# stecrotti/MPSKit.jl

Hardware: AMD Instinct MI355X
Metric: DMRG sweeps/sec + ddAC matvec achieved-TFLOP/s, Heisenberg L=100 D=1024 fp64 (higher is better)
Workload: dtype f64; 1 GPU; Heisenberg S=1/2 FiniteMPS L=100 D=1024 d=2 W=5 fp64, 1-site DMRG sweep (2L-2 site updates), fixed Krylov budget 8 matvecs/site; parallelism=single GPU

## Files before the change

### include/mpsk.h

```cpp
#ifndef MPSK_H
#define MPSK_H
#include <stddef.h>
#include <stdint.h>

#ifdef __cplusplus
extern "C" {
#endif

typedef struct mpsk_ctx mpsk_ctx;
typedef struct mpsk_mposlice mpsk_mposlice;

enum { MPSK_F64 = 0, MPSK_C128 = 1 };
enum { MPSK_OK = 0, MPSK_ERR_INVALID = 1, MPSK_ERR_HIP = 2, MPSK_ERR_UNSUPPORTED = 3, MPSK_ERR_NOMEM = 4 };
enum { MPSK_BLOCK_ZERO = 0, MPSK_BLOCK_SCALAR = 1, MPSK_BLOCK_DENSE = 2 };

int mpsk_version(void);
const char* mpsk_last_error(void);

int mpsk_ctx_create(int device, mpsk_ctx** out);
int mpsk_ctx_destroy(mpsk_ctx* ctx);
int mpsk_ctx_set_stream(mpsk_ctx* ctx, void* hip_stream);
int mpsk_ctx_set_dtype(mpsk_ctx* ctx, int dtype);
int mpsk_ctx_get_stream(mpsk_ctx* ctx, void** hip_stream);
int mpsk_ctx_get_device(mpsk_ctx* ctx, int* device);
// ... 32 lines not shown
                    mpsk_hac** out);
enum { MPSK_HAC_CANONICAL = 1 };
int mpsk_hac_create_ex(mpsk_ctx* ctx, const mpsk_mposlice* H, int Dlo, int Dl, int Dr, const void* GL, const void* GR,
                       int flags, mpsk_hac** out);
int mpsk_hac_apply(mpsk_hac* h, const void* x, int nblk, void* y);
int mpsk_hac_eigsolve_fixed(mpsk_hac* hac, const void* x0, int m, void* const* V, void* scal, void* y, void* first_image);
int mpsk_hac_destroy(mpsk_hac* h);
int mpsk_hac_info(const mpsk_hac* h, int* mode, int* nslabs);
int mpsk_dC(mpsk_ctx* ctx, int W, int Dlo, int Dl, int Dr, const void* GL, const void* GR,
            const void* c, void* y);
int mpsk_dAC2(mpsk_ctx* ctx, const mpsk_mposlice* H1, const mpsk_mposlice* H2, int Dlo, int Dl, int Dr,
              const void* GL, const void* GR, const void* x2, void* y2);

int mpsk_dAC2_product(mpsk_ctx* ctx, const mpsk_mposlice* H1, const mpsk_mposlice* H2, int Dl, int Dm, int Dr,
                      const void* GL, const void* GR, const void* AC, const void* AR, void* Y);
int mpsk_complement_tsvd(mpsk_ctx* ctx, int m, int n, const void* Y, int ldy, const void* QL, int ldql, int pl,
                         const void* QR, int ldqr, int pr, int k, void* U, int ldu, void* S, void* Vt, int ldvt, int* kept);
int mpsk_ctx_complement_stats(mpsk_ctx* ctx, long* n_calls, long* n_subspace, long* n_full);

int mpsk_transfer_left(mpsk_ctx* ctx, const mpsk_mposlice* H, int W, int d, int Dl, int Dr, int Dlb,
                       int Drb, const void* GLin, const void* A, const void* Ab, void* GLout);
int mpsk_transfer_right(mpsk_ctx* ctx, const mpsk_mposlice* H, int W, int d, int Dl, int Dr, int Dlb,
                        int Drb, const void* A, const void* Ab, const void* GRin, void* GRout);
int mpsk_regularize(mpsk_ctx* ctx, int W, int D1, int D2, void* v, const void* lvec, const void* rvec);

int mpsk_qrpos(mpsk_ctx* ctx, int m, int n, const void* A, int lda, void* Q, int ldq, void* R, int ldr);
int mpsk_qrpos2(mpsk_ctx* ctx, int m, int n, const void* A1, int lda1, void* Q1, int ldq1, void* R1, int ldr1,
                const void* A2, int lda2, void* Q2, int ldq2, void* R2, int ldr2);
int mpsk_qrlq_pair(mpsk_ctx* ctx, int m, int n, const void* A1, int lda1, void* Q1, int ldq1, void* R1, int ldr1,
                   const void* A2, int lda2, void* L2, int ldl2, void* Q2, int ldq2);
int mpsk_lqpos(mpsk_ctx* ctx, int m, int n, const void* A, int lda, void* L, int ldl, void* Q, int ldq);
int mpsk_ctx_qr_defer(mpsk_ctx* ctx);
int mpsk_ctx_side_mark(mpsk_ctx* ctx);
int mpsk_ctx_side_begin(mpsk_ctx* ctx);
int mpsk_ctx_side_end(mpsk_ctx* ctx);
int mpsk_qr_commit(mpsk_ctx* ctx, int* redone);
int mpsk_tsvd(mpsk_ctx* ctx, int m, int n, const void* theta, int ldt, void* U, int ldu, void* S, void* Vh,
              int ldv, int max_keep, double trunc_err, int* kept, double* disc_norm);
int mpsk_tsplit(mpsk_ctx* ctx, int m, int n, const void* theta, int ldt, int max_keep, double trunc_err,
                void* AL, int ldal, void* C, int ldc, void* AR, int ldar, void* S, int* kept, double* disc_norm);
int mpsk_cx_embed(mpsk_ctx* ctx, int m, int n, const void* H, int64_t ldh, void* E, int64_t lde);
int mpsk_cx_half(mpsk_ctx* ctx, int m, int n, const void* E, int64_t lde, void* H, int64_t ldh);
int mpsk_gemm(mpsk_ctx* ctx, int transA, int transB, int M, int N, int K, double alpha, const void* A,
              int64_t lda, const void* B, int64_t ldb, double beta, void* C, int64_t ldc);

int mpsk_copy2d(mpsk_ctx* ctx, int rows, int cols, const void* src, int64_t lds, void* dst, int64_t ldd);
// ... 25 lines not shown
```

### mpskit.jl_amd/_lib.py

```python
from __future__ import annotations

import ctypes as C
import os

_HERE = os.path.dirname(os.path.abspath(__file__))
LIB_PATH = os.environ.get("MPSK_LIB") or os.path.join(_HERE, "libmpsk.so")


class MpskError(RuntimeError):
    pass


_lib = None

c_void_pp = C.POINTER(C.c_void_p)
c_int32_p = C.POINTER(C.c_int32)
c_double_p = C.POINTER(C.c_double)

SIGNATURES = {
    "mpsk_ctx_create": [C.c_int, c_void_pp],
    "mpsk_ctx_destroy": [C.c_void_p],
    "mpsk_ctx_set_stream": [C.c_void_p, C.c_void_p],
    "mpsk_ctx_synchronize": [C.c_void_p],
    "mpsk_ctx_workspace_reserve": [C.c_void_p, C.c_size_t],
# ... 15 lines not shown
    "mpsk_mposlice_create_dense": [C.c_void_p, C.c_int, C.c_int, C.c_int, C.c_int, C.c_void_p, c_void_pp],
    "mpsk_mposlice_destroy": [C.c_void_p],
    "mpsk_mposlice_dims": [C.c_void_p, C.POINTER(C.c_int), C.POINTER(C.c_int), C.POINTER(C.c_int)],
    "mpsk_dAC": [C.c_void_p, C.c_void_p, C.c_int, C.c_int, C.c_int, C.c_void_p, C.c_void_p, C.c_void_p,
                 C.c_void_p],
    "mpsk_dAC_blocked": [C.c_void_p, C.c_void_p, C.c_int, C.c_int, C.c_int, C.c_int, C.c_void_p, C.c_void_p,
                         C.c_void_p, C.c_void_p],
    "mpsk_ctx_set_dtype": [C.c_void_p, C.c_int],
    "mpsk_ctx_get_stream": [C.c_void_p, c_void_pp],
    "mpsk_ctx_get_device": [C.c_void_p, C.POINTER(C.c_int)],
    "mpsk_hac_create": [C.c_void_p, C.c_void_p, C.c_int, C.c_int, C.c_int, C.c_void_p, C.c_void_p, c_void_pp],
    "mpsk_hac_create_ex": [C.c_void_p, C.c_void_p, C.c_int, C.c_int, C.c_int, C.c_void_p, C.c_void_p, C.c_int, c_void_pp],
    "mpsk_hac_apply": [C.c_void_p, C.c_void_p, C.c_int, C.c_void_p],
    "mpsk_hac_destroy": [C.c_void_p],
    "mpsk_hac_info": [C.c_void_p, C.POINTER(C.c_int), C.POINTER(C.c_int)],
    "mpsk_dC": [C.c_void_p, C.c_int, C.c_int, C.c_int, C.c_int, C.c_void_p, C.c_void_p, C.c_void_p,
                C.c_void_p],
    "mpsk_dAC2": [C.c_void_p, C.c_void_p, C.c_void_p, C.c_int, C.c_int, C.c_int, C.c_void_p, C.c_void_p,
                  C.c_void_p, C.c_void_p],
    "mpsk_transfer_left": [C.c_void_p, C.c_void_p, C.c_int, C.c_int, C.c_int, C.c_int, C.c_int, C.c_int,
                           C.c_void_p, C.c_void_p, C.c_void_p, C.c_void_p],
    "mpsk_transfer_right": [C.c_void_p, C.c_void_p, C.c_int, C.c_int, C.c_int, C.c_int, C.c_int, C.c_int,
                            C.c_void_p, C.c_void_p, C.c_void_p, C.c_void_p],
    "mpsk_regularize": [C.c_void_p, C.c_int, C.c_int, C.c_int, C.c_void_p, C.c_void_p, C.c_void_p],
    "mpsk_qrpos": [C.c_void_p, C.c_int, C.c_int, C.c_void_p, C.c_int, C.c_void_p, C.c_int, C.c_void_p, C.c_int],
    "mpsk_qrpos2": [C.c_void_p, C.c_int, C.c_int, C.c_void_p, C.c_int, C.c_void_p, C.c_int, C.c_void_p, C.c_int,
                    C.c_void_p, C.c_int, C.c_void_p, C.c_int, C.c_void_p, C.c_int],
    "mpsk_qrlq_pair": [C.c_void_p, C.c_int, C.c_int, C.c_void_p, C.c_int, C.c_void_p, C.c_int, C.c_void_p, C.c_int,
                       C.c_void_p, C.c_int, C.c_void_p, C.c_int, C.c_void_p, C.c_int],
    "mpsk_lqpos": [C.c_void_p, C.c_int, C.c_int, C.c_void_p, C.c_int, C.c_void_p, C.c_int, C.c_void_p, C.c_int],
    "mpsk_tsvd": [C.c_void_p, C.c_int, C.c_int, C.c_void_p, C.c_int, C.c_void_p, C.c_int, C.c_void_p,
                  C.c_void_p, C.c_int, C.c_int, C.c_double, C.POINTER(C.c_int), c_double_p],
    "mpsk_tsplit": [C.c_void_p, C.c_int, C.c_int, C.c_void_p, C.c_int, C.c_int, C.c_double, C.c_void_p, C.c_int,
                    C.c_void_p, C.c_int, C.c_void_p, C.c_int, C.c_void_p, C.POINTER(C.c_int), c_double_p],
    "mpsk_gemm": [C.c_void_p, C.c_int, C.c_int, C.c_int, C.c_int, C.c_int, C.c_double, C.c_void_p,
                  C.c_int64, C.c_void_p, C.c_int64, C.c_double, C.c_void_p, C.c_int64],
    "mpsk_copy2d": [C.c_void_p, C.c_int, C.c_int, C.c_void_p, C.c_int64, C.c_void_p, C.c_int64],
    "mpsk_vdot": [C.c_void_p, C.c_int64, C.c_void_p, C.c_void_p, c_double_p],
    "mpsk_vnrm2": [C.c_void_p, C.c_int64, C.c_void_p, c_double_p],
    "mpsk_vaxpby": [C.c_void_p, C.c_int64, C.c_double, C.c_void_p, C.c_double, C.c_void_p],
    "mpsk_vscal": [C.c_void_p, C.c_int64, C.c_double, C.c_void_p],
    "mpsk_vtimes_i": [C.c_void_p, C.c_int64, C.c_void_p, C.c_void_p],
    "mpsk_vcopy": [C.c_void_p, C.c_int64, C.c_void_p, C.c_void_p],
    "mpsk_vzero": [C.c_void_p, C.c_int64, C.c_void_p],
    "mpsk_vmultidot": [C.c_void_p, C.c_int64, C.c_int, c_void_pp, C.c_void_p, c_double_p],
    "mpsk_vgs_step": [C.c_void_p, C.c_int64, C.c_int, c_void_pp, C.c_void_p, c_double_p],
# ... 95 lines not shown
```

### mpskit.jl_amd/backend.py

```python
from __future__ import annotations

import ctypes as C
import numpy as np

from . import _lib
from ._lib import MpskError, check


def _torch():
    import torch
    return torch


class DTensor:
    __slots__ = ("buf", "shape")

    def __init__(self, buf, shape):
        self.buf = buf
        self.shape = tuple(int(s) for s in shape)

    @property
    def ptr(self):
        return self.buf.data_ptr()

# ... 247 lines not shown
              "mpsk_dAC2_product")
        return y

    def complement_tsvd(self, Y: DTensor, QL: DTensor, QR: DTensor, k: int):
        m, n = Y.shape
        pl = 0 if QL is None else QL.shape[1]
        pr = 0 if QR is None else QR.shape[0]
        kk = max(0, min(int(k), m - pl, n - pr))
        U, S, Vt = self.empty(m, kk), self.empty(kk), self.empty(kk, n)
        kept = C.c_int(-1)
        check(self.lib.mpsk_complement_tsvd(self.ctx, m, n, Y.ptr, m, None if QL is None else QL.ptr, m, pl,
                                            None if QR is None else QR.ptr, max(pr, 1), pr, int(k), U.ptr, m, S.ptr, Vt.ptr,
                                            max(kk, 1), C.byref(kept)), "mpsk_complement_tsvd")
        assert kept.value == kk, (kept.value, kk)
        if kk == 0:
            return None, None, None, 0
        return U, S, Vt, kk

    def complement_stats(self):
        a, b, c = C.c_long(), C.c_long(), C.c_long()
        check(self.lib.mpsk_ctx_complement_stats(self.ctx, C.byref(a), C.byref(b), C.byref(c)), "mpsk_ctx_complement_stats")
        return {"calls": a.value, "subspace": b.value, "full": c.value}

    def transfer_left(self, H, GLin: DTensor, A: DTensor, Ab: DTensor, out: DTensor = None, cplx=False):
        if cplx or getattr(H, "cplx", False):
            Dl, d, Dr = A.shape[0] // 2, A.shape[1], A.shape[2]
            Dlb, Drb = Ab.shape[0] // 2, Ab.shape[2]
            W = GLin.shape[0]
            Wout = H.Wr if H is not None else W
            y = self.empty(Wout, 2 * Drb, Dr) if out is None else out
            if H is None:
                self._set_dtype(True)
            try:
                check(self.lib.mpsk_transfer_left(self.ctx, H.handle if H is not None else None, W, d, Dl, Dr, Dlb, Drb,
                                                  GLin.ptr, A.ptr, Ab.ptr, y.ptr), "mpsk_transfer_left")
            finally:
                if H is None:
                    self._set_dtype(False)
            return y
        Dl, d, Dr = A.shape
        Dlb, _, Drb = Ab.shape
        W = GLin.shape[0]
        Wout = H.Wr if H is not None else W
        y = self.empty(Wout, Drb, Dr) if out is None else out
        check(self.lib.mpsk_transfer_left(self.ctx, H.handle if H is not None else None, W, d, Dl, Dr, Dlb, Drb,
                                          GLin.ptr, A.ptr, Ab.ptr, y.ptr), "mpsk_transfer_left")
        return y

    def transfer_right(self, H, GRin: DTensor, A: DTensor, Ab: DTensor, out: DTensor = None, cplx=False):
        if cplx or getattr(H, "cplx", False):
            Dl, d, Dr = A.shape[0] // 2, A.shape[1], A.shape[2]
            Dlb, Drb = Ab.shape[0] // 2, Ab.shape[2]
            W = GRin.shape[0]
            Wout = H.Wl if H is not None else W
            y = self.empty(Wout, 2 * Dl, Dlb) if out is None else out
            if H is None:
                self._set_dtype(True)
            try:
                check(self.lib.mpsk_transfer_right(self.ctx, H.handle if H is not None else None, W, d, Dl, Dr, Dlb, Drb,
                                                   A.ptr, Ab.ptr, GRin.ptr, y.ptr), "mpsk_transfer_right")
            finally:
                if H is None:
                    self._set_dtype(False)
            return y
        Dl, d, Dr = A.shape
        Dlb, _, Drb = Ab.shape
        W = GRin.shape[0]
        Wout = H.Wl if H is not None else W
        y = self.empty(Wout, Dl, Dlb) if out is None else out
        check(self.lib.mpsk_transfer_right(self.ctx, H.handle if H is not None else None, W, d, Dl, Dr, Dlb, Drb,
                                           A.ptr, Ab.ptr, GRin.ptr, y.ptr), "mpsk_transfer_right")
        return y

    def regularize(self, v: DTensor, lvec: DTensor, rvec: DTensor):
        W, D1, D2 = v.shape
        check(self.lib.mpsk_regularize(self.ctx, W, D1, D2, v.ptr, lvec.ptr, rvec.ptr), "mpsk_regularize")
        return v

    def gemm(self, A: DTensor, B: DTensor, transA=False, transB=False, alpha=1.0, beta=0.0, out: DTensor = None,
             m=None, n=None, k=None, lda=None, ldb=None, ldc=None):
        ar, ac = A.shape
        br, bc = B.shape
        M = (ac if transA else ar) if m is None else m
        K = (ar if transA else ac) if k is None else k
        N = (br if transB else bc) if n is None else n
        c = self.empty(M, N) if out is None else out
        check(self.lib.mpsk_gemm(self.ctx, int(transA), int(transB), M, N, K, float(alpha), A.ptr,
                                 ar if lda is None else lda, B.ptr, br if ldb is None else ldb, float(beta),
                                 c.ptr, M if ldc is None else ldc), "mpsk_gemm")
        return c

    def gemm_raw(self, transA, transB, M, N, K, alpha, a_ptr, lda, b_ptr, ldb, beta, c_ptr, ldc):
# ... 459 lines not shown
```

### mpskit.jl_amd/csrc/mpsk_api.hip

```cpp
#include <hip/hip_runtime.h>
#include <cstdio>
#include <cstdlib>
#include <cstring>
#include <cmath>
#include <algorithm>
#include <map>
#include <string>
#include <vector>
#include "mpsk.h"
#include "mpsk_internal.h"

using namespace mpsk;

static thread_local std::string g_err;
static int fail(int code, const std::string& msg) { g_err = msg; return code; }
#define HIPCHK(expr)                                                                        \
  do {                                                                                      \
    hipError_t e_ = (expr);                                                                 \
    if (e_ != hipSuccess)                                                                   \
      return fail(MPSK_ERR_HIP, std::string(#expr) + ": " + hipGetErrorString(e_));         \
  } while (0)
#define REQUIRE(cond, msg)                                                  \
  do {                                                                      \
    if (!(cond)) return fail(MPSK_ERR_INVALID, std::string(__func__) + ": " + (msg)); \
// ... 1 lines not shown

static constexpr int MPSK_DENSE_MIN_CHID = 8;

struct mpsk_mposlice {
  mpsk_ctx* ctx;
  int Wl, Wr, d;
  int dtype = MPSK_F64;
  std::vector<double> Ofull;
  std::vector<double> Ofull_im;
  MixPlan fwd;
  MixPlan bwd;
  MixPlan rgt;
  double Oi(int w, int t, int s, int v) const {
    return Ofull_im.empty() ? 0.0 : Ofull_im[w + (size_t)Wl * (t + d * (s + (size_t)d * v))];
  }
  std::vector<char> row_used, col_used;
  MixPlan rc;
  std::vector<int> rc_w, rc_s, rc_t;
  int rc_nseg = 0;
  bool jordan = false;
  MixPlan jr, jl;
  std::vector<int> jr_p, jl_p;
  int jr_nseg = 0, jl_nseg = 0;
  double O(int w, int t, int s, int v) const { return Ofull[w + (size_t)Wl * (t + d * (s + (size_t)d * v))]; }
  bool dense = false;
  double* d_Od = nullptr;
  mutable std::map<std::pair<int64_t, int64_t>, int64_t*> dtab;
  double* d_OdR = nullptr;
  mutable std::map<std::pair<int64_t, int64_t>, int64_t*> dtabR;
};

struct PoolBuf { void* p; size_t bytes; bool used; hipStream_t last = nullptr; hipEvent_t ev = nullptr; bool ev_set = false; };

struct mpsk_ctx {
  int device = 0;
  hipStream_t stream = nullptr;
  void* ws = nullptr;
  size_t ws_bytes = 0;
  double* d_scal = nullptr;
  double* d_partial = nullptr;
  double* h_scal = nullptr;
  double* d_coef = nullptr;
  double* h_coef = nullptr;
  hipEvent_t ev_coef = nullptr;
  bool coef_pending = false;
  int dtype = MPSK_F64;
// ... 329 lines not shown
            if (s->O(0, t, si, v) != 0.0) { jr.push_back({p, v, s->O(0, t, si, v)}); r_used[p] = 1; }
          for (int w = 1; w < Wl; ++w)
            if (s->O(w, t, si, Wr - 1) != 0.0) { jl.push_back({p, w, s->O(w, t, si, Wr - 1)}); l_used[p] = 1; }
        }
      auto lists = [&](const std::vector<char>& used, std::vector<int>& out, int& nseg) {
        int empty = -1;
        for (int p = 0; p < d * d; ++p) if (!used[p]) { empty = p; break; }
        for (int t = 0; t < d; ++t) {
          int n = 0;
          for (int si = 0; si < d; ++si) n += used[si + d * t];
          nseg = std::max(nseg, n);
        }
        out.assign((size_t)d * nseg, empty);
        for (int t = 0; t < d; ++t) {
          int k = 0;
          for (int si = 0; si < d; ++si) if (used[si + d * t]) out[(size_t)t * nseg + k++] = si + d * t;
        }
      };
      lists(r_used, s->jr_p, s->jr_nseg);
      lists(l_used, s->jl_p, s->jl_nseg);
      HIPCHK(mix_plan_create(jr, d * d, Wr, &s->jr));
      HIPCHK(mix_plan_create(jl, d * d, Wl, &s->jl));
      s->jordan = s->jr_nseg > 0 && s->jl_nseg > 0;
    }
  }
  if (dense) {
    const int Wl = s->Wl, Wr = s->Wr;
    std::vector<double> od((size_t)d * Wl * d * Wr);
    for (int v = 0; v < Wr; ++v)
      for (int t = 0; t < d; ++t)
        for (int w = 0; w < Wl; ++w)
          for (int si = 0; si < d; ++si)
            od[(si + (size_t)d * w) + (size_t)d * Wl * (t + (size_t)d * v)] = s->O(w, t, si, v);
    s->dense = true;
    if (hipMalloc(&s->d_Od, sizeof(double) * od.size()) != hipSuccess) { mpsk_mposlice_destroy(s); return fail(MPSK_ERR_NOMEM, "dense MPO hipMalloc failed"); }
    HIPCHK(hipMemcpy(s->d_Od, od.data(), sizeof(double) * od.size(), hipMemcpyHostToDevice));
    for (int v = 0; v < Wr; ++v)
      for (int t = 0; t < d; ++t)
        for (int w = 0; w < Wl; ++w)
          for (int si = 0; si < d; ++si)
            od[(si + (size_t)d * v) + (size_t)d * Wr * (t + (size_t)d * w)] = s->O(w, t, si, v);
    if (hipMalloc(&s->d_OdR, sizeof(double) * od.size()) != hipSuccess) { mpsk_mposlice_destroy(s); return fail(MPSK_ERR_NOMEM, "dense MPO hipMalloc failed"); }
    HIPCHK(hipMemcpy(s->d_OdR, od.data(), sizeof(double) * od.size(), hipMemcpyHostToDevice));
  }
  *out = s;
  return MPSK_OK;
// ... 10 lines not shown
  REQUIRE(dtype == MPSK_F64, "dense MPO slices are MPSK_F64 only (complex DenseMPO is not implemented; build an MPSK_C128 "
                             "slice with mpsk_mposlice_create instead)");
  REQUIRE(Wl > 0 && Wr > 0 && d > 0, "Wl, Wr and d must be positive");
  const int32_t cl = Wl, cr = Wr, kind = MPSK_BLOCK_DENSE;
  const void* blocks[1] = {O};
  return mposlice_build(c, dtype, 1, &cl, &cr, d, &kind, nullptr, blocks, true, out);
}

int mpsk_mposlice_destroy(mpsk_mposlice* s) {
  if (!s) return MPSK_OK;
  mpsk_ctx* c = s->ctx;
  (void)hipSetDevice(c->device);
  (void)hipStreamSynchronize(c->stream);
  for (auto it = c->pair_plans.begin(); it != c->pair_plans.end();) {
    if (it->first.first == s || it->first.second == s) { mix_plan_destroy(&it->second); it = c->pair_plans.erase(it); }
    else ++it;
  }
  mix_plan_destroy(&s->fwd);
  mix_plan_destroy(&s->bwd);
  mix_plan_destroy(&s->rgt);
  mix_plan_destroy(&s->rc);
  mix_plan_destroy(&s->jr);
  mix_plan_destroy(&s->jl);
  if (s->d_Od) (void)hipFree(s->d_Od);
  if (s->d_OdR) (void)hipFree(s->d_OdR);
  for (auto& kv : s->dtab) (void)hipFree(kv.second);
  for (auto& kv : s->dtabR) (void)hipFree(kv.second);
  delete s;
  return MPSK_OK;
}

int mpsk_mposlice_dims(const mpsk_mposlice* s, int* Wl, int* Wr, int* d) {
  REQUIRE(s, "slice is NULL");
  if (Wl) *Wl = s->Wl;
  if (Wr) *Wr = s->Wr;
  if (d) *d = s->d;
  return MPSK_OK;
}

}

static int ensure_ws(mpsk_ctx* c, size_t bytes) {
  if (c->pend.active) return fail(MPSK_ERR_INVALID, "a deferred factorization still owns the workspace: call mpsk_qr_commit first");
  if (c->on_side) return fail(MPSK_ERR_INVALID, "workspace users are not accepted on the side stream: call mpsk_ctx_side_end first");
  if (bytes <= c->ws_bytes) return MPSK_OK;
  return mpsk_ctx_workspace_reserve(c, bytes + bytes / 4);
// ... 665 lines not shown
  HIPCHK(hipSetDevice(c->device));
  const int d1 = H1->d, d2 = H2->d, Wl = H1->Wl, Wr = H2->Wr;
  const size_t plane = (size_t)Dlo * d1 * Dr;
  const size_t slab = plane * d2;
  if (int rc = ensure_ws(c, sizeof(double) * slab * (Wl + Wr))) return rc;
  double* T1 = (double*)c->ws;
  double* T2 = T1 + slab * Wl;
  const MixPlan* plan = nullptr;
  if (int rc = pair_plan(c, H1, H2, &plan)) return rc;
  GemmArgs g1 = mk((const double*)GL, (const double*)x2, T1, Dlo, d1 * Dr * d2, Dl, Dlo, Dl, Dlo);
  g1.batch = Wl; g1.bsA = (int64_t)Dlo * Dl; g1.bsB = 0; g1.bsC = (int64_t)slab;
  g1.tag = 1;
  HIPCHK(gemm_f64(g1, c->stream));
  SlabIndex ix{d1, d2, (int64_t)Dlo, (int64_t)plane, (int64_t)slab, (int64_t)Dlo * d1};
  HIPCHK(mix_apply(*plan, T1, ix, T2, ix, Dlo, Dr, c->stream));
  std::vector<int64_t> sa, sb;
  for (int v = 0; v < Wr; ++v) if (H2->col_used[v]) { sa.push_back((int64_t)v * slab); sb.push_back((int64_t)v * Dr * Dr); }
  if (sa.empty()) { HIPCHK(zero_async(y2, sizeof(double) * slab, c->stream)); return MPSK_OK; }
  GemmArgs g3 = mk(T2, (const double*)GR, (double*)y2, Dlo * d1, Dr, Dr, (int64_t)Dlo * d1, Dr, (int64_t)Dlo * d1);
  g3.tag = 1;
  g3.batch = d2; g3.bsA = (int64_t)plane; g3.bsB = 0; g3.bsC = (int64_t)plane;
  HIPCHK(gemm_segments(g3, sa, sb, c->stream));
  return MPSK_OK;
}

int mpsk_transfer_left(mpsk_ctx* c, const mpsk_mposlice* H, int W, int d, int Dl, int Dr, int Dlb, int Drb,
                       const void* GLin, const void* A, const void* Ab, void* GLout) {
  REQUIRE(c && GLin && A && Ab && GLout, "NULL argument");
  HIPCHK(hipSetDevice(c->device));
  int Wl = W, Wr = W;
  if (H) { Wl = H->Wl; Wr = H->Wr; d = H->d; }
  REQUIRE(Wl > 0 && d > 0 && Dl > 0 && Dr > 0 && Dlb > 0 && Drb > 0, "dimensions must be positive");
  if ((H ? H->dtype : c->dtype) == MPSK_C128)
    return transfer_left_c128(c, H, W, d, Dl, Dr, Dlb, Drb, (const double*)GLin, (const double*)A, (const double*)Ab, (double*)GLout);
  if (dense_route(H))
    return transfer_left_dense(c, H, Dl, Dr, Dlb, Drb, (const double*)GLin, (const double*)A, (const double*)Ab, (double*)GLout);
  const size_t slab = (size_t)Dlb * d * Dr;
  if (int rc = ensure_ws(c, sizeof(double) * slab * (Wl + (H ? Wr : 0)))) return rc;
  double* T1 = (double*)c->ws;
  double* T2 = H ? T1 + slab * Wl : T1;
  GemmArgs g1 = mk((const double*)GLin, (const double*)A, T1, Dlb, d * Dr, Dl, Dlb, Dl, Dlb);
  g1.batch = Wl; g1.bsA = (int64_t)Dlb * Dl; g1.bsB = 0; g1.bsC = (int64_t)slab;
  HIPCHK(gemm_f64(g1, c->stream));
  if (H) {
    SlabIndex ix{d, 1 << 30, (int64_t)Dlb, (int64_t)slab, 0, (int64_t)Dlb * d};
    HIPCHK(mix_apply(H->fwd, T1, ix, T2, ix, Dlb, Dr, c->stream));
// ... 1563 lines not shown
```

### mpskit.jl_amd/csrc/mpsk_internal.h

```cpp
#pragma once
#include <hip/hip_runtime.h>
#include <stdint.h>
#include <stddef.h>
#include <atomic>
#include <vector>
#include <string>

namespace mpsk {

inline hipError_t ensure_dyn_smem(std::atomic<uint64_t>& done, const void* kernel, size_t bytes) {
  int dev = 0;
  hipError_t e = hipGetDevice(&dev);
  if (e != hipSuccess) return e;
  const uint64_t bit = 1ull << (dev & 63);
  if (done.load(std::memory_order_acquire) & bit) return hipSuccess;
  e = hipFuncSetAttribute(kernel, hipFuncAttributeMaxDynamicSharedMemorySize, (int)bytes);
  if (e != hipSuccess) return e;
  done.fetch_or(bit, std::memory_order_release);
  return hipSuccess;
}

constexpr int MAXSEG = 32;

struct GemmArgs {
// ... 41 lines not shown
std::string gemm_prof_summary();

struct MixTerm { int32_t out, in; double coef; double coef_im = 0.0; };

struct MixPlan {
  int n_out = 0, n_in = 0;
  int32_t* d_rowptr = nullptr;
  int32_t* d_src = nullptr;
  double* d_coef = nullptr;
  double* d_coef_im = nullptr;
  int nnz = 0;
  int max_terms = 0;
};

hipError_t mix_plan_create(const std::vector<MixTerm>& terms, int n_out, int n_in, MixPlan* plan);
void mix_plan_destroy(MixPlan* plan);

struct SlabIndex { int n0, n1; int64_t s0, s1, s2; int64_t ld; };
hipError_t mix_apply(const MixPlan& plan, const double* in, SlabIndex iin, double* out, SlabIndex iout,
                     int R, int C, hipStream_t s);
hipError_t deinterleave(const double* z, int64_t n, double* re, double* im, hipStream_t s);
hipError_t copy_strided(const double* src, int64_t srs, int64_t scs, double* dst, int64_t drs, int64_t dcs, int64_t R,
                        int64_t C, hipStream_t s);

constexpr int MPSK_DOT_SCRATCH = 32 * 1024;
hipError_t vec_multidot(const double* const* xs, int k, const double* y, int64_t n, double* d_out,
                        double* d_partial, hipStream_t s);
hipError_t vec_axpby(double a, const double* x, double b, double* y, int64_t n, hipStream_t s);
hipError_t vec_times_i(const double* x, double* y, int64_t n, hipStream_t s);
hipError_t vec_scal(double a, double* x, int64_t n, hipStream_t s);
hipError_t vec_scal_rsqrt_dev(const double* d_n2, double* x, int64_t n, hipStream_t s);
hipError_t vec_scal_rsqrt_dev_oop(const double* d_n2, const double* x, double* y, int64_t n, hipStream_t s);
hipError_t vec_cgs2(const double* const* xs, int k, double* y, int64_t n, double* d_out, double* d_partial, hipStream_t s);
hipError_t vec_ritz_small(const double* d_slot, int m, int stride, double* d_coef, double* d_info, hipStream_t s);
hipError_t vec_multilincomb(const double* const* xs, int k, double* const* ys, int m, const double* d_coefs, int64_t n,
                            hipStream_t s);
hipError_t vec_multiaxpy(const double* const* xs, const double* d_coefs, int k, double sign, double* y,
                         int64_t n, hipStream_t s);

size_t regularize_workspace_doubles(int W, int D1, int D2);
hipError_t regularize(int W, int D1, int D2, double* v, const double* lvec, const double* rvec, double* partial, hipStream_t s);
hipError_t transpose(const double* in, int ldi, int rows, int cols, double* out, int ldo, hipStream_t s);
size_t qrpos_workspace_doubles(int m, int n);
hipError_t qrpos(int m, int n, const double* A, int lda, double* Q, int ldq, double* R, int ldr, double* ws,
                 hipStream_t s, std::string* err);

// ... 23 lines not shown
```

### mpskit.jl_amd/csrc/mpsk_ops.hip

```cpp
#include <hip/hip_runtime.h>
#include "mpsk_internal.h"

namespace mpsk {

typedef double d2 __attribute__((ext_vector_type(2)));

__device__ inline int64_t slab_off(const SlabIndex& ix, int j) {
  int j0 = j % ix.n0;
  int t = j / ix.n0;
  int j1 = t % ix.n1;
  int j2 = t / ix.n1;
  return j0 * ix.s0 + j1 * ix.s1 + j2 * ix.s2;
}

template <bool VEC2>
__global__ __launch_bounds__(256) void mix_kernel(const int32_t* __restrict__ rowptr,
                                                  const int32_t* __restrict__ src,
                                                  const double* __restrict__ coef,
                                                  const double* __restrict__ coef_im,
                                                  const double* __restrict__ in, SlabIndex iin,
                                                  double* __restrict__ out, SlabIndex iout, int R, int C) {
  const int o = blockIdx.y;
  const int t0 = rowptr[o], t1 = rowptr[o + 1];
  double* op = out + slab_off(iout, o);
// ... 105 lines not shown
}
__global__ __launch_bounds__(256) void deinterleave_kernel(const d2* __restrict__ z, double* __restrict__ re,
                                                           double* __restrict__ im, int64_t n) {
  for (int64_t e = blockIdx.x * (int64_t)blockDim.x + threadIdx.x; e < n; e += (int64_t)gridDim.x * blockDim.x) {
    const d2 v = z[e];
    re[e] = v.x;
    im[e] = v.y;
  }
}
hipError_t deinterleave(const double* z, int64_t n, double* re, double* im, hipStream_t s) {
  if (n <= 0) return hipSuccess;
  int64_t nb = (n + 255) / 256;
  if (nb > 4096) nb = 4096;
  hipLaunchKernelGGL(deinterleave_kernel, dim3((unsigned)nb), dim3(256), 0, s, reinterpret_cast<const d2*>(z), re, im, n);
  return hipGetLastError();
}

hipError_t copy_strided(const double* src, int64_t srs, int64_t scs, double* dst, int64_t drs, int64_t dcs, int64_t R,
                        int64_t C, hipStream_t s) {
  if (R <= 0 || C <= 0) return hipSuccess;
  int64_t nb = (R * C + 255) / 256;
  if (nb > 4096) nb = 4096;
  hipLaunchKernelGGL(copy_strided_kernel, dim3((unsigned)nb), dim3(256), 0, s, src, srs, scs, dst, drs, dcs, R, C);
  return hipGetLastError();
}

__device__ inline double wave_sum(double v) {
#pragma unroll
  for (int off = 32; off > 0; off >>= 1) v += __shfl_down(v, off, 64);
  return v;
}

template <int NV> __device__ inline void block_sum(double (&v)[NV], double* sh ) {
  const int lane = threadIdx.x & 63, wave = threadIdx.x >> 6;
#pragma unroll
  for (int i = 0; i < NV; ++i) {
    double w = wave_sum(v[i]);
    if (lane == 0) sh[wave * NV + i] = w;
  }
  __syncthreads();
  if (threadIdx.x == 0) {
#pragma unroll
    for (int i = 0; i < NV; ++i) v[i] = sh[i] + sh[NV + i] + sh[2 * NV + i] + sh[3 * NV + i];
  }
  __syncthreads();
}
// ... 503 lines not shown
```

### mpskit.jl_amd/environments.py

```python
from __future__ import annotations

import numpy as np

from .backend import Backend, DTensor
from . import krylov


def _start_env(be: Backend, chis, D, active_level):
    W = sum(chis)
    host = np.zeros((W, D, D))
    off = 0
    for i, chi in enumerate(chis):
        if i == active_level:
            for k in range(chi):
                host[off + k] = np.eye(D)
        off += chi
    t = be.upload(np.transpose(host, (1, 2, 0)))
    return DTensor(t.buf, (W, D, D))


class FinEnv:

    def __init__(self, psi, H):
        be = self.be = psi.be
        L = len(psi)
        self.H = H
        self.opp = [H[i] for i in range(L)]
        odim = H.odim
        D0 = psi.AL(0).shape[0]
        t = psi.ARs[L - 1] if psi.ARs[L - 1] is not None else psi.AL(L - 1)
        DL = t.shape[2]
        self.leftenvs = [_start_env(be, self.opp[0].chil, D0, 0)] + [None] * L
        self.rightenvs = [None] * L + [_start_env(be, self.opp[L - 1].chir, DL, odim - 1)]
        self.ldeps = [None] * L
        self.rdeps = [None] * L
        self.n_transfers = 0

    def rightenv(self, ind, psi):
        L = len(psi)
        a = None
        for i in range(L - 1, ind, -1):
            if psi.AR(i) is not self.rdeps[i]:
                a = i
                break
        if a is not None:
            for j in range(a, ind, -1):
                ar = psi.AR(j)
                self.rightenvs[j] = self.be.transfer_right(self.opp[j], self.rightenvs[j + 1], ar, ar)
                self.rdeps[j] = ar
                self.n_transfers += 1
        return self.rightenvs[ind + 1]

    def leftenv(self, ind, psi):
        a = None
        for i in range(0, ind):
            if psi.AL(i) is not self.ldeps[i]:
                a = i
                break
        if a is not None:
            for j in range(a, ind):
                al = psi.AL(j)
                self.leftenvs[j + 1] = self.be.transfer_left(self.opp[j], self.leftenvs[j], al, al)
                self.ldeps[j] = al
                self.n_transfers += 1
        return self.leftenvs[ind]

    def poison(self, ind):
        self.ldeps[ind] = None
        self.rdeps[ind] = None


class MultipleEnvironments:

    def __init__(self, H, envs):
        self.H, self.envs = H, list(envs)

    def recalculate(self, psi, tol=None):
        for e in self.envs:
            e.recalculate(psi, tol)
        return self


def environments(psi, H, **kw):
    from .states import FiniteMPS
    from .operators import LazySum
    from .statmech import DenseMPO, PerMPOInfEnv
    if isinstance(H, DenseMPO):
        return PerMPOInfEnv(psi, H, **kw)
    if isinstance(H, LazySum):
        return MultipleEnvironments(H, [environments(psi, h, **kw) for h in H])
    if isinstance(psi, FiniteMPS):
        return FinEnv(psi, H)
    return MPOHamInfEnv(psi, H, **kw)


class MPOHamInfEnv:

    def __init__(self, psi, H, tol=1e-12, maxiter=100, rng=None):
# ... 194 lines not shown
```

Baseline: 1.094 sweeps/s.

## Add canonical-gauge environment transfers exploiting Jordan MPO structure and isometry

Adds specialised left/right environment transfer paths for f64 Jordan-form MPOs on canonical (isometric) tensors. They write the identity block directly instead of computing it, and fold the sparse Jordan terms into segmented batched GEMMs plus small mix kernels. Finite-MPS environments use these paths by default. The cost is extra code paths whose correctness relies on the tensors actually being isometric, which is only checked when a debug environment variable is set.

Result: faster. 1.153 sweeps/s, median of 6 (+5.4%).

```diff
diff --git a/include/mpsk.h b/include/mpsk.h
--- a/include/mpsk.h
+++ b/include/mpsk.h
@@ -78,6 +78,11 @@
                        int Drb, const void* GLin, const void* A, const void* Ab, void* GLout);
 int mpsk_transfer_right(mpsk_ctx* ctx, const mpsk_mposlice* H, int W, int d, int Dl, int Dr, int Dlb,
                         int Drb, const void* A, const void* Ab, const void* GRin, void* GRout);
+enum { MPSK_TRANSFER_CANONICAL = 1 };
+int mpsk_transfer_left_ex(mpsk_ctx* ctx, const mpsk_mposlice* H, int W, int d, int Dl, int Dr, int Dlb, int Drb,
+                          const void* GLin, const void* A, const void* Ab, int flags, void* GLout);
+int mpsk_transfer_right_ex(mpsk_ctx* ctx, const mpsk_mposlice* H, int W, int d, int Dl, int Dr, int Dlb, int Drb,
+                           const void* A, const void* Ab, const void* GRin, int flags, void* GRout);
 int mpsk_regularize(mpsk_ctx* ctx, int W, int D1, int D2, void* v, const void* lvec, const void* rvec);
 
 int mpsk_qrpos(mpsk_ctx* ctx, int m, int n, const void* A, int lda, void* Q, int ldq, void* R, int ldr);
diff --git a/mpskit.jl_amd/_lib.py b/mpskit.jl_amd/_lib.py
--- a/mpskit.jl_amd/_lib.py
+++ b/mpskit.jl_amd/_lib.py
@@ -61,6 +61,10 @@
                            C.c_void_p, C.c_void_p, C.c_void_p, C.c_void_p],
     "mpsk_transfer_right": [C.c_void_p, C.c_void_p, C.c_int, C.c_int, C.c_int, C.c_int, C.c_int, C.c_int,
                             C.c_void_p, C.c_void_p, C.c_void_p, C.c_void_p],
+    "mpsk_transfer_left_ex": [C.c_void_p, C.c_void_p, C.c_int, C.c_int, C.c_int, C.c_int, C.c_int, C.c_int,
+                              C.c_void_p, C.c_void_p, C.c_void_p, C.c_int, C.c_void_p],
+    "mpsk_transfer_right_ex": [C.c_void_p, C.c_void_p, C.c_int, C.c_int, C.c_int, C.c_int, C.c_int, C.c_int,
+                               C.c_void_p, C.c_void_p, C.c_void_p, C.c_int, C.c_void_p],
     "mpsk_regularize": [C.c_void_p, C.c_int, C.c_int, C.c_int, C.c_void_p, C.c_void_p, C.c_void_p],
     "mpsk_qrpos": [C.c_void_p, C.c_int, C.c_int, C.c_void_p, C.c_int, C.c_void_p, C.c_int, C.c_void_p, C.c_int],
     "mpsk_qrpos2": [C.c_void_p, C.c_int, C.c_int, C.c_void_p, C.c_int, C.c_void_p, C.c_int, C.c_void_p, C.c_int,
diff --git a/mpskit.jl_amd/backend.py b/mpskit.jl_amd/backend.py
--- a/mpskit.jl_amd/backend.py
+++ b/mpskit.jl_amd/backend.py
@@ -293,7 +293,7 @@
         check(self.lib.mpsk_ctx_complement_stats(self.ctx, C.byref(a), C.byref(b), C.byref(c)), "mpsk_ctx_complement_stats")
         return {"calls": a.value, "subspace": b.value, "full": c.value}
 
-    def transfer_left(self, H, GLin: DTensor, A: DTensor, Ab: DTensor, out: DTensor = None, cplx=False):
+    def transfer_left(self, H, GLin: DTensor, A: DTensor, Ab: DTensor, out: DTensor = None, cplx=False, canonical=False):
         if cplx or getattr(H, "cplx", False):
             Dl, d, Dr = A.shape[0] // 2, A.shape[1], A.shape[2]
             Dlb, Drb = Ab.shape[0] // 2, Ab.shape[2]
@@ -314,11 +314,21 @@
         W = GLin.shape[0]
         Wout = H.Wr if H is not None else W
         y = self.empty(Wout, Drb, Dr) if out is None else out
+        if canonical and H is not None:
+            check(self.lib.mpsk_transfer_left_ex(self.ctx, H.handle, W, d, Dl, Dr, Dlb, Drb, GLin.ptr, A.ptr, Ab.ptr, 1, y.ptr),
+                  "mpsk_transfer_left_ex")
+            return y
         check(self.lib.mpsk_transfer_left(self.ctx, H.handle if H is not None else None, W, d, Dl, Dr, Dlb, Drb,
                                           GLin.ptr, A.ptr, Ab.ptr, y.ptr), "mpsk_transfer_left")
         return y
 
-    def transfer_right(self, H, GRin: DTensor, A: DTensor, Ab: DTensor, out: DTensor = None, cplx=False):
+    def transfer_left_ex(self, H, GLin: DTensor, A: DTensor, Ab: DTensor, canonical: bool = False, out: DTensor = None):
+        return self.transfer_left(H, GLin, A, Ab, out=out, canonical=canonical)
+
+    def transfer_right_ex(self, H, GRin: DTensor, A: DTensor, Ab: DTensor, canonical: bool = False, out: DTensor = None):
+        return self.transfer_right(H, GRin, A, Ab, out=out, canonical=canonical)
+
+    def transfer_right(self, H, GRin: DTensor, A: DTensor, Ab: DTensor, out: DTensor = None, cplx=False, canonical=False):
         if cplx or getattr(H, "cplx", False):
             Dl, d, Dr = A.shape[0] // 2, A.shape[1], A.shape[2]
             Dlb, Drb = Ab.shape[0] // 2, Ab.shape[2]
@@ -339,6 +349,10 @@
         W = GRin.shape[0]
         Wout = H.Wl if H is not None else W
         y = self.empty(Wout, Dl, Dlb) if out is None else out
+        if canonical and H is not None:
+            check(self.lib.mpsk_transfer_right_ex(self.ctx, H.handle, W, d, Dl, Dr, Dlb, Drb, A.ptr, Ab.ptr, GRin.ptr, 1, y.ptr),
+                  "mpsk_transfer_right_ex")
+            return y
         check(self.lib.mpsk_transfer_right(self.ctx, H.handle if H is not None else None, W, d, Dl, Dr, Dlb, Drb,
                                            A.ptr, Ab.ptr, GRin.ptr, y.ptr), "mpsk_transfer_right")
         return y
diff --git a/mpskit.jl_amd/csrc/mpsk_api.hip b/mpskit.jl_amd/csrc/mpsk_api.hip
--- a/mpskit.jl_amd/csrc/mpsk_api.hip
+++ b/mpskit.jl_amd/csrc/mpsk_api.hip
@@ -47,6 +47,10 @@
   MixPlan jr, jl;
   std::vector<int> jr_p, jl_p;
   int jr_nseg = 0, jl_nseg = 0;
+  MixPlan tl, tr;
+  bool tl_dblock = false;
+  mutable std::map<int64_t, int64_t*> jtabL;
+  mutable std::map<std::pair<int64_t, int64_t>, int64_t*> jtabR;
   double O(int w, int t, int s, int v) const { return Ofull[w + (size_t)Wl * (t + d * (s + (size_t)d * v))]; }
   bool dense = false;
   double* d_Od = nullptr;
@@ -422,6 +426,18 @@
       HIPCHK(mix_plan_create(jr, d * d, Wr, &s->jr));
       HIPCHK(mix_plan_create(jl, d * d, Wl, &s->jl));
       s->jordan = s->jr_nseg > 0 && s->jl_nseg > 0;
+      if (s->jordan) {
+        std::vector<MixTerm> tl, tr;
+        for (int t = 0; t < d; ++t)
+          for (int si = 0; si < d; ++si) {
+            for (int v = 1; v < Wr; ++v)
+              if (s->O(0, t, si, v) != 0.0) { tl.push_back({t + d * (v - 1), si, s->O(0, t, si, v)}); if (v == Wr - 1) s->tl_dblock = true; }
+            for (int w = 1; w < Wl - 1; ++w)
+              if (s->O(w, t, si, Wr - 1) != 0.0) tr.push_back({t + d * (w - 1), si, s->O(w, t, si, Wr - 1)});
+          }
+        HIPCHK(mix_plan_create(tl, d * (Wr - (s->tl_dblock ? 1 : 2)), d, &s->tl));
+        HIPCHK(mix_plan_create(tr, d * (Wl - 2), d, &s->tr));
+      }
     }
   }
   if (dense) {
@@ -478,6 +494,10 @@
   mix_plan_destroy(&s->rc);
   mix_plan_destroy(&s->jr);
   mix_plan_destroy(&s->jl);
+  mix_plan_destroy(&s->tl);
+  mix_plan_destroy(&s->tr);
+  for (auto& kv : s->jtabL) (void)hipFree(kv.second);
+  for (auto& kv : s->jtabR) (void)hipFree(kv.second);
   if (s->d_Od) (void)hipFree(s->d_Od);
   if (s->d_OdR) (void)hipFree(s->d_OdR);
   for (auto& kv : s->dtab) (void)hipFree(kv.second);
@@ -1189,6 +1209,157 @@
   g3.batch = d2; g3.bsA = (int64_t)plane; g3.bsB = 0; g3.bsC = (int64_t)plane;
   HIPCHK(gemm_segments(g3, sa, sb, c->stream));
   return MPSK_OK;
+}
+
+static size_t up32(size_t n) { return (n + 31) & ~(size_t)31; }
+
+static bool transfer_canonical_ok(const mpsk_mposlice* H, int flags, const void* A, const void* Ab, int Dl, int Dr,
+                                  int Dlb, int Drb) {
+  if (!(flags & MPSK_TRANSFER_CANONICAL) || !H || !H->jordan || H->dtype != MPSK_F64 || dense_route(H)) return false;
+  if (A != Ab || Dl != Dlb || Dr != Drb) return false;
+  const char* ev = getenv("MPSK_TRANSFER_MODE");
+  return !(ev && ev[0] == '0');
+}
+
+static bool hac_check_on() { const char* ev = getenv("MPSK_HAC_CHECK"); return ev && ev[0] == '1'; }
+
+static int transfer_canonical_check(mpsk_ctx* c, const char* who, const double* G, int n, const double* A, int d, int Dl,
+                                    int Dr, bool left) {
+  double dg = 0.0, da = 0.0;
+  if (int rc = identity_deviation(c, G, n, &dg)) return rc;
+  const int m = left ? Dr : Dl;
+  if (int rc = ensure_ws(c, sizeof(double) * (size_t)m * m)) return rc;
+  double* gram = (double*)c->ws;
+  if (left) {
+    GemmArgs g = mk(A, A, gram, Dr, Dr, Dl * d, (int64_t)Dl * d, (int64_t)Dl * d, Dr, 1, 0);
+    HIPCHK(gemm_f64(g, c->stream));
+  } else {
+    std::vector<int64_t> sa;
+    for (int t = 0; t < d; ++t) sa.push_back((int64_t)t * Dl);
+    GemmArgs g = mk(A, A, gram, Dl, Dl, Dr, (int64_t)Dl * d, (int64_t)Dl * d, Dl, 0, 1);
+    HIPCHK(gemm_segments(g, sa, sa, c->stream));
+  }
+  if (int rc = identity_deviation(c, gram, m, &da)) return rc;
+  if (!(dg <= 1e-10 && da <= 1e-10)) {
+    char msg[200];
+    snprintf(msg, sizeof(msg), "MPSK_HAC_CHECK: %s is not canonical (max|G[identity level] - I| = %.3e, max|%s - I| = %.3e)",
+             who, dg, left ? "A^T A" : "A A^T", da);
+    return fail(MPSK_ERR_INVALID, msg);
+  }
+  return MPSK_OK;
+}
+
+static int jordan_tab(const mpsk_mposlice* H, bool left, int Dl, int Dr, const int64_t** out) {
+  if (left) { auto it = H->jtabL.find(Dl); if (it != H->jtabL.end()) { *out = it->second; return MPSK_OK; } }
+  else { auto it = H->jtabR.find({Dl, Dr}); if (it != H->jtabR.end()) { *out = it->second; return MPSK_OK; } }
+  const int d = H->d, n = left ? H->jl_nseg : H->jr_nseg;
+  const std::vector<int>& plist = left ? H->jl_p : H->jr_p;
+  const int64_t tL = (int64_t)Dl * d * Dl, tR = (int64_t)Dr * d * Dr;
+  std::vector<int64_t> h((size_t)2 * d * n);
+  for (int t = 0; t < d; ++t)
+    for (int k = 0; k < n; ++k) {
+      const int p = plist[(size_t)t * n + k], si = p % d, tt = p / d;
+      if (left) { h[(size_t)t * n + k] = tt * tL + (int64_t)si * Dl; h[(size_t)(d + t) * n + k] = (int64_t)si * Dl; }
+      else { h[(size_t)t * n + k] = (int64_t)si * Dl; h[(size_t)(d + t) * n + k] = tt * tR + (int64_t)si * Dr; }
+    }
+  int64_t* p = nullptr;
+  if (hipMalloc(&p, sizeof(int64_t) * h.size()) != hipSuccess) return fail(MPSK_ERR_NOMEM, "transfer segment table hipMalloc failed");
+  if (hipMemcpy(p, h.data(), sizeof(int64_t) * h.size(), hipMemcpyHostToDevice) != hipSuccess) {
+    (void)hipFree(p);
+    return fail(MPSK_ERR_HIP, "transfer segment table upload failed");
+  }
+  if (left) H->jtabL.emplace(Dl, p); else H->jtabR.emplace(std::make_pair((int64_t)Dl, (int64_t)Dr), p);
+  *out = p;
+  return MPSK_OK;
+}
+
+static int transfer_left_canonical(mpsk_ctx* c, const mpsk_mposlice* H, int Dl, int Dr, const double* GLin, const double* A,
+                                   double* GLout) {
+  const int d = H->d, Wr = H->Wr, n2 = H->jl_nseg;
+  if (hac_check_on())
+    if (int rc = transfer_canonical_check(c, "mpsk_transfer_left_ex", GLin, Dl, A, d, Dl, Dr, true)) return rc;
+  const size_t slab = (size_t)Dl * d * Dr;
+  const int64_t tL = (int64_t)Dl * d * Dl;
+  const size_t nL = up32((size_t)d * tL);
+  if (int rc = ensure_ws(c, sizeof(double) * (nL + slab * (Wr - 1)))) return rc;
+  const int64_t* tab = nullptr;
+  if (int rc = jordan_tab(H, true, Dl, Dr, &tab)) return rc;
+  double* GLc = (double*)c->ws;
+  double* T2 = GLc + nL;
+  double* T = T2 + slab * (Wr - 2);
+  SlabIndex il{1 << 30, 1, (int64_t)Dl * Dl, 0, 0, (int64_t)Dl}, ol{d, 1 << 30, (int64_t)Dl, tL, 0, (int64_t)d * Dl};
+  HIPCHK(mix_apply(H->jl, GLin, il, GLc, ol, Dl, Dl, c->stream));
+  SlabIndex ia{1 << 30, 1, (int64_t)Dl, 0, 0, (int64_t)Dl * d}, ot{d, 1 << 30, (int64_t)Dl, (int64_t)slab, 0, (int64_t)Dl * d};
+  HIPCHK(mix_apply(H->tl, A, ia, T2, ot, Dl, Dr, c->stream));
+  GemmArgs g = mk(GLc, A, T, Dl, Dr, Dl, (int64_t)Dl * d, (int64_t)Dl * d, (int64_t)Dl * d);
+  g.batch = d; g.bsA = 0; g.bsB = 0; g.bsC = (int64_t)Dl;
+  g.beta = H->tl_dblock ? 1.0 : 0.0;
+  g.nseg = n2; g.zsegA = tab; g.zsegB = tab + (size_t)d * n2;
+  g.tabs_even = Dl % 2 == 0;
+  g.tag = 1;
+  HIPCHK(gemm_f64(g, c->stream));
+  HIPCHK(identity_slab(GLout, Dr, c->stream));
+  GemmArgs g3 = mk(A, T2, GLout + (size_t)Dr * Dr, Dr, Dr, Dl * d, (int64_t)Dl * d, (int64_t)Dl * d, Dr, 1, 0);
+  g3.batch = Wr - 1; g3.bsA = 0; g3.bsB = (int64_t)slab; g3.bsC = (int64_t)Dr * Dr;
+  HIPCHK(gemm_f64(g3, c->stream));
+  return MPSK_OK;
+}
+
+static int transfer_right_canonical(mpsk_ctx* c, const mpsk_mposlice* H, int Dl, int Dr, const double* A, const double* GRin,
+                                    double* GRout) {
+  const int d = H->d, Wl = H->Wl, Wr = H->Wr, n1 = H->jr_nseg;
+  if (hac_check_on())
+    if (int rc = transfer_canonical_check(c, "mpsk_transfer_right_ex", GRin + (size_t)(Wr - 1) * Dr * Dr, Dr, A, d, Dl, Dr, false))
+      return rc;
+  const size_t slab = (size_t)Dl * d * Dr;
+  const int64_t tR = (int64_t)Dr * d * Dr;
+  const size_t nR = up32((size_t)d * tR);
+  if (int rc = ensure_ws(c, sizeof(double) * (nR + slab * (Wl - 1)))) return rc;
+  const int64_t* tab = nullptr;
+  if (int rc = jordan_tab(H, false, Dl, Dr, &tab)) return rc;
+  double* GRc = (double*)c->ws;
+  double* X = GRc + nR;
+  SlabIndex ir{1 << 30, 1, (int64_t)Dr * Dr, 0, 0, (int64_t)Dr}, orr{d, 1 << 30, (int64_t)Dr, tR, 0, (int64_t)d * Dr};
+  HIPCHK(mix_apply(H->jr, GRin, ir, GRc, orr, Dr, Dr, c->stream));
+  SlabIndex ia{1 << 30, 1, (int64_t)Dl, 0, 0, (int64_t)Dl * d}, ox{d, 1 << 30, (int64_t)Dl, (int64_t)slab, 0, (int64_t)Dl * d};
+  HIPCHK(mix_apply(H->tr, A, ia, X + slab, ox, Dl, Dr, c->stream));
+  GemmArgs g = mk(A, GRc, X, Dl, Dr, Dr, (int64_t)Dl * d, (int64_t)Dr * d, (int64_t)Dl * d);
+  g.batch = d; g.bsA = 0; g.bsB = 0; g.bsC = (int64_t)Dl;
+  g.nseg = n1; g.zsegA = tab; g.zsegB = tab + (size_t)d * n1;
+  g.tabs_even = Dl % 2 == 0 && Dr % 2 == 0;
+  g.tag = 1;
+  HIPCHK(gemm_f64(g, c->stream));
+  HIPCHK(identity_slab(GRout + (size_t)(Wl - 1) * Dl * Dl, Dl, c->stream));
+  std::vector<int64_t> sa;
+  for (int t = 0; t < d; ++t) sa.push_back((int64_t)t * Dl);
+  GemmArgs g3 = mk(X, A, GRout, Dl, Dl, Dr, (int64_t)Dl * d, (int64_t)Dl * d, Dl, 0, 1);
+  g3.batch = Wl - 1; g3.bsA = (int64_t)slab; g3.bsB = 0; g3.bsC = (int64_t)Dl * Dl;
+  HIPCHK(gemm_segments(g3, sa, sa, c->stream));
+  return MPSK_OK;
+}
+
+int mpsk_transfer_left_ex(mpsk_ctx* c, const mpsk_mposlice* H, int W, int d, int Dl, int Dr, int Dlb, int Drb,
+                          const void* GLin, const void* A, const void* Ab, int flags, void* GLout) {
+  REQUIRE(c && GLin && A && Ab && GLout, "NULL argument");
+  REQUIRE((flags & ~MPSK_TRANSFER_CANONICAL) == 0, "unknown flags");
+  if (transfer_canonical_ok(H, flags, A, Ab, Dl, Dr, Dlb, Drb)) {
+    REQUIRE(Dl > 0 && Dr > 0, "dimensions must be positive");
+    HIPCHK(hipSetDevice(c->device));
+    return transfer_left_canonical(c, H, Dl, Dr, (const double*)GLin, (const double*)A, (double*)GLout);
+  }
+  return mpsk_transfer_left(c, H, W, d, Dl, Dr, Dlb, Drb, GLin, A, Ab, GLout);
+}
+
+int mpsk_transfer_right_ex(mpsk_ctx* c, const mpsk_mposlice* H, int W, int d, int Dl, int Dr, int Dlb, int Drb,
+                           const void* A, const void* Ab, const void* GRin, int flags, void* GRout) {
+  REQUIRE(c && GRin && A && Ab && GRout, "NULL argument");
+  REQUIRE((flags & ~MPSK_TRANSFER_CANONICAL) == 0, "unknown flags");
+  if (transfer_canonical_ok(H, flags, A, Ab, Dl, Dr, Dlb, Drb)) {
+    REQUIRE(Dl > 0 && Dr > 0, "dimensions must be positive");
+    HIPCHK(hipSetDevice(c->device));
+    return transfer_right_canonical(c, H, Dl, Dr, (const double*)A, (const double*)GRin, (double*)GRout);
+  }
+  return mpsk_transfer_right(c, H, W, d, Dl, Dr, Dlb, Drb, A, Ab, GRin, GRout);
 }
 
 int mpsk_transfer_left(mpsk_ctx* c, const mpsk_mposlice* H, int W, int d, int Dl, int Dr, int Dlb, int Drb,
diff --git a/mpskit.jl_amd/csrc/mpsk_internal.h b/mpskit.jl_amd/csrc/mpsk_internal.h
--- a/mpskit.jl_amd/csrc/mpsk_internal.h
+++ b/mpskit.jl_amd/csrc/mpsk_internal.h
@@ -87,6 +87,7 @@
 hipError_t deinterleave(const double* z, int64_t n, double* re, double* im, hipStream_t s);
 hipError_t copy_strided(const double* src, int64_t srs, int64_t scs, double* dst, int64_t drs, int64_t dcs, int64_t R,
                         int64_t C, hipStream_t s);
+hipError_t identity_slab(double* G, int n, hipStream_t s);
 
 constexpr int MPSK_DOT_SCRATCH = 32 * 1024;
 hipError_t vec_multidot(const double* const* xs, int k, const double* y, int64_t n, double* d_out,
diff --git a/mpskit.jl_amd/csrc/mpsk_ops.hip b/mpskit.jl_amd/csrc/mpsk_ops.hip
--- a/mpskit.jl_amd/csrc/mpsk_ops.hip
+++ b/mpskit.jl_amd/csrc/mpsk_ops.hip
@@ -151,6 +151,19 @@
   int64_t nb = (R * C + 255) / 256;
   if (nb > 4096) nb = 4096;
   hipLaunchKernelGGL(copy_strided_kernel, dim3((unsigned)nb), dim3(256), 0, s, src, srs, scs, dst, drs, dcs, R, C);
+  return hipGetLastError();
+}
+
+__global__ __launch_bounds__(256) void identity_slab_kernel(double* __restrict__ G, int n) {
+  const int64_t total = (int64_t)n * n;
+  for (int64_t e = blockIdx.x * (int64_t)blockDim.x + threadIdx.x; e < total; e += (int64_t)gridDim.x * blockDim.x)
+    G[e] = (e % n == e / n) ? 1.0 : 0.0;
+}
+hipError_t identity_slab(double* G, int n, hipStream_t s) {
+  if (n <= 0) return hipSuccess;
+  int64_t nb = ((int64_t)n * n + 255) / 256;
+  if (nb > 4096) nb = 4096;
+  hipLaunchKernelGGL(identity_slab_kernel, dim3((unsigned)nb), dim3(256), 0, s, G, n);
   return hipGetLastError();
 }
 
diff --git a/mpskit.jl_amd/environments.py b/mpskit.jl_amd/environments.py
--- a/mpskit.jl_amd/environments.py
+++ b/mpskit.jl_amd/environments.py
@@ -35,6 +35,11 @@
         self.ldeps = [None] * L
         self.rdeps = [None] * L
         self.n_transfers = 0
+        self.canonical = True
+
+    def _canonical(self, psi):
+        return (self.canonical and type(self) is FinEnv and not getattr(psi, "cplx", False)
+                and hasattr(self.be, "transfer_left_ex"))
 
     def rightenv(self, ind, psi):
         L = len(psi)
@@ -44,9 +49,10 @@
                 a = i
                 break
         if a is not None:
+            kw = {"canonical": True} if self._canonical(psi) else {}
             for j in range(a, ind, -1):
                 ar = psi.AR(j)
-                self.rightenvs[j] = self.be.transfer_right(self.opp[j], self.rightenvs[j + 1], ar, ar)
+                self.rightenvs[j] = self.be.transfer_right(self.opp[j], self.rightenvs[j + 1], ar, ar, **kw)
                 self.rdeps[j] = ar
                 self.n_transfers += 1
         return self.rightenvs[ind + 1]
@@ -58,9 +64,10 @@
                 a = i
                 break
         if a is not None:
+            kw = {"canonical": True} if self._canonical(psi) else {}
             for j in range(a, ind):
                 al = psi.AL(j)
-                self.leftenvs[j + 1] = self.be.transfer_left(self.opp[j], self.leftenvs[j], al, al)
+                self.leftenvs[j + 1] = self.be.transfer_left(self.opp[j], self.leftenvs[j], al, al, **kw)
                 self.ldeps[j] = al
                 self.n_transfers += 1
         return self.leftenvs[ind]
@@ -74,6 +81,9 @@
 
     def __init__(self, H, envs):
         self.H, self.envs = H, list(envs)
+        for e in self.envs:
+            if isinstance(e, FinEnv):
+                e.canonical = False
 
     def recalculate(self, psi, tol=None):
         for e in self.envs:
```
